# lainy/sdrangel

Measured on AMD Instinct MI355X. Metric: MS/s complex int16 IQ through decim-64 + DownChannelizer, 1/2/4/8 GPU; % HBM roofline, higher is better.
Workload: dtype int32

## Files before the change

sdrangel_amd/csrc/sdrx_chan.hip:

```cpp
#include "sdrx_common.hpp"
#include "chan_plan.hpp"
#include "tree_kernel.hpp"
#include "tree_mx_kernel.hpp"
#include <vector>
#include <cstring>
#include <new>
#include <algorithm>
#include "chan_plan.cpp"
#include "chan_lower.cpp"

using namespace sdrx;

namespace {

struct Channel {
    int32_t out_rate = 0, ofs = 0;
    int n = 0;
    uint8_t modes[32] = { 0 };
    int group = -1;
    bool passthrough = false;
    bool dead = false;
    DevBuf out;
    int64_t avail = 0;
    int64_t last_off = 0, last_n = 0;
};

struct StreamBuf {
    uint32_t* hist[2] = { nullptr, nullptr };
    int cur = 0;
    DevBuf mid;
};

struct Group {
    int index = -1;
    int64_t T = 0;
    std::vector<int> chans;
    BankPlan plan;
    LoweredBank low;
    std::vector<StreamBuf> bufs;
    void* d_static = nullptr;
    TkSubtree* d_subtrees = nullptr; TkNode* d_nodes = nullptr; TkArray* d_arrays = nullptr; TkMJob* d_mjobs = nullptr;
    TkLJob* d_ljobs = nullptr;
};

}

struct sdrx_chan_bank {
    int device = 0, cus = 256;
    int32_t in_rate = 0;
    hipStream_t own_stream = nullptr, stream = nullptr;
    std::vector<Channel> ch;
    std::vector<Group*> groups;
    DevBuf stage_in;
    DevBuf scratch;
    static constexpr int RING = 4;
    void* h_dyn[RING] = { nullptr, nullptr, nullptr, nullptr };
    void* d_dyn[RING] = { nullptr, nullptr, nullptr, nullptr };
    size_t dyn_cap[RING] = { 0, 0, 0, 0 };
    hipEvent_t dyn_ev[RING] = { nullptr, nullptr, nullptr, nullptr };
    int dyn_next = 0;
    char last_name[96] = "";
    int last_grid = 0, last_block = 0, last_lds = 0;
    EventTimer timer;
};

static void free_group(Group* g)
{
    if (!g) return;
    for (auto& s : g->bufs) { for (uint32_t* h : s.hist) if (h) (void)hipFree(h); s.mid.release(); }
    if (g->d_static) (void)hipFree(g->d_static);
    delete g;
}

static int upload_group(sdrx_chan_bank* b, Group* g)
{
    const BankPlan& p = g->plan;
    g->bufs.resize(p.streams.size());
    for (size_t si = 0; si < p.streams.size(); si++) {
        const size_t bytes = (size_t)p.streams[si].hist_len * 4;
        for (uint32_t*& h : g->bufs[si].hist) {
            SDRX_HIP(hipMalloc(reinterpret_cast<void**>(&h), bytes));
            SDRX_HIP(hipMemsetAsync(h, 0, bytes, b->stream));
        }
    }
    const size_t b0 = p.subtrees.size() * sizeof(TkSubtree), b1 = p.nodes.size() * sizeof(TkNode), b2 = p.arrays.size() * sizeof(TkArray);
    const size_t b3 = p.mjobs.size() * sizeof(TkMJob), b4 = g->low.jobs.size() * sizeof(TkLJob);
    if (b0 + b1 + b2 == 0) return SDRX_OK;
    SDRX_HIP(hipMalloc(&g->d_static, b0 + b1 + b2 + b3 + b4 + 64));
    char* d = static_cast<char*>(g->d_static);
    g->d_subtrees = reinterpret_cast<TkSubtree*>(d);
    g->d_nodes = reinterpret_cast<TkNode*>(d + b0);
    g->d_arrays = reinterpret_cast<TkArray*>(d + b0 + b1);
    g->d_mjobs = reinterpret_cast<TkMJob*>(d + b0 + b1 + b2);
    g->d_ljobs = reinterpret_cast<TkLJob*>(d + b0 + b1 + b2 + b3);
    if (b0) SDRX_HIP(hipMemcpy(g->d_subtrees, p.subtrees.data(), b0, hipMemcpyHostToDevice));
    if (b1) SDRX_HIP(hipMemcpy(g->d_nodes, p.nodes.data(), b1, hipMemcpyHostToDevice));
    if (b2) SDRX_HIP(hipMemcpy(g->d_arrays, p.arrays.data(), b2, hipMemcpyHostToDevice));
    if (b3) SDRX_HIP(hipMemcpy(g->d_mjobs, p.mjobs.data(), b3, hipMemcpyHostToDevice));
    if (b4) SDRX_HIP(hipMemcpy(g->d_ljobs, g->low.jobs.data(), b4, hipMemcpyHostToDevice));
    return SDRX_OK;
}

static int configure_channel(sdrx_chan_bank* b, int c, int32_t req_rate, int32_t req_fc)
{
    Channel& ch = b->ch[c];
    ch.n = plan_chain(b->in_rate, req_rate, req_fc, ch.modes, MAX_STAGES, &ch.out_rate, &ch.ofs);
    ch.passthrough = ch.n == 0;
    return SDRX_OK;
}

static int new_group(sdrx_chan_bank* b, const std::vector<int>& chans)
{
    if (chans.empty()) return SDRX_OK;
    std::vector<PlanChain> chains;
    for (int c : chans) chains.push_back(PlanChain{ c, b->ch[(size_t)c].n, b->ch[(size_t)c].modes });
    BankPlan plan;
    const std::string err = plan_bank(chains, plan_options_from_env(), plan);
    if (!err.empty()) { set_error(err); return SDRX_EINVAL; }
    LoweredBank low;
    (void)lower_bank(plan, low);
    Group* g = new (std::nothrow) Group;
    if (!g) return SDRX_ENOMEM;
    g->chans = chans;
    g->index = (int)b->groups.size();
    g->plan = std::move(plan);
    g->low = std::move(low);
    int rc = upload_group(b, g);
    if (rc) { free_group(g); return rc; }
    for (int c : chans) b->ch[c].group = g->index;
    b->groups.push_back(g);
    return SDRX_OK;
}

static int retire_dead_groups(sdrx_chan_bank* b)
{
    for (size_t gi = 0; gi < b->groups.size();) {
        Group* g = b->groups[gi];
        bool live = false;
        for (int c : g->chans) if (b->ch[(size_t)c].group == g->index) { live = true; break; }
        if (live) { gi++; continue; }
        SDRX_HIP(hipStreamSynchronize(b->stream));
        free_group(g);
        b->groups.erase(b->groups.begin() + (long)gi);
        for (size_t k = gi; k < b->groups.size(); k++) {
            const int old = b->groups[k]->index;
            b->groups[k]->index = (int)k;
            for (int c : b->groups[k]->chans) if (b->ch[(size_t)c].group == old) b->ch[(size_t)c].group = (int)k;
        }
    }
    return SDRX_OK;
}

static int grow_keep(sdrx_chan_bank* b, DevBuf& buf, size_t used, size_t need)
{
    if (need <= buf.cap) return SDRX_OK;
    size_t want = buf.cap ? buf.cap : (1 << 16);
    while (want < need) want *= 2;
    void* np = nullptr;
    SDRX_HIP(hipMalloc(&np, want));
    if (used) SDRX_HIP(hipMemcpyAsync(np, buf.p, used, hipMemcpyDeviceToDevice, b->stream));
    SDRX_HIP(hipStreamSynchronize(b->stream));
    if (buf.p) (void)hipFree(buf.p);
    buf.p = np; buf.cap = want;
    return SDRX_OK;
}

static int dyn_slot(sdrx_chan_bank* b, size_t bytes, int* slot)
{
    const int s = b->dyn_next; b->dyn_next = (b->dyn_next + 1) % sdrx_chan_bank::RING;
    if (b->dyn_ev[s]) SDRX_HIP(hipEventSynchronize(b->dyn_ev[s]));
    else SDRX_HIP(hipEventCreateWithFlags(&b->dyn_ev[s], hipEventDisableTiming));
    if (bytes > b->dyn_cap[s]) {
        size_t want = b->dyn_cap[s] ? b->dyn_cap[s] : 4096; while (want < bytes) want *= 2;
        if (b->h_dyn[s]) (void)hipHostFree(b->h_dyn[s]);
        if (b->d_dyn[s]) (void)hipFree(b->d_dyn[s]);
        b->h_dyn[s] = b->d_dyn[s] = nullptr; b->dyn_cap[s] = 0;
        SDRX_HIP(hipHostMalloc(&b->h_dyn[s], want, hipHostMallocDefault));
        SDRX_HIP(hipMalloc(&b->d_dyn[s], want));
        b->dyn_cap[s] = want;
    }
    *slot = s;
    return SDRX_OK;
}

static int feed_group(sdrx_chan_bank* b, Group* g, const uint32_t* d_in, int64_t n)
{
    const int64_t T0 = g->T, T1 = g->T + n;
    for (int c : g->chans) {
        Channel& ch = b->ch[c];
        if (ch.group != g->index) continue;
        const int64_t add = (T1 >> ch.n) - (T0 >> ch.n);
        int rc = grow_keep(b, ch.out, (size_t)ch.avail * 4, (size_t)(ch.avail + add) * 4 + 64); if (rc) return rc;
    }
    const BankPlan& plan = g->plan;
    for (size_t si = 1; si < plan.streams.size(); si++) {
        const int64_t add = (T1 >> plan.streams[si].depth) - (T0 >> plan.streams[si].depth);
        int rc = g->bufs[si].mid.reserve((size_t)add * 4 + 64); if (rc) return rc;
    }
    const size_t ns = plan.streams.size(), nk = plan.sinks.size();
    const size_t o_sinks = ns * sizeof(TkStream), o_hist = o_sinks + nk * sizeof(TkSink), total = o_hist + ns * sizeof(TkHistJob);
    int slot; int rc = dyn_slot(b, total, &slot); if (rc) return rc;
    char* hp = static_cast<char*>(b->h_dyn[slot]); char* dp = static_cast<char*>(b->d_dyn[slot]);
    TkStream* hs = reinterpret_cast<TkStream*>(hp);
    TkSink* hk = reinterpret_cast<TkSink*>(hp + o_sinks);
    TkHistJob* hh = reinterpret_cast<TkHistJob*>(hp + o_hist);

    std::vector<long> segs(ns, 0);
    for (size_t si = 0; si < ns; si++) {
        const PlanStream& s = plan.streams[si];
        const StreamBuf& sb = g->bufs[si];
        TkStream& t = hs[si];
        t.hist = sb.hist[sb.cur];
        t.in = si == 0 ? d_in : static_cast<const uint32_t*>(sb.mid.p);
        t.t_old = T0 >> s.depth; t.t_new = T1 >> s.depth;
        t.subtree = s.subtree;
        t.c_first = t.t_old / TK_CHUNK;
        t.c_last = t.t_new > t.t_old ? (t.t_new - 1) / TK_CHUNK : t.c_first - 1;
        t.cps = 1;
        t.hist_len = s.hist_len;
        hh[si] = TkHistJob{ sb.hist[sb.cur], t.in, sb.hist[sb.cur ^ 1], t.t_new - t.t_old, s.hist_len };
    }
    for (size_t k = 0; k < nk; k++) {
        const PlanSink& si = plan.sinks[k];
        TkSink& t = hk[k];
        t.shift = 0; t.next = si.next;
        if (si.kind == 0) {
            Channel& ch = b->ch[si.ch];
            t.lo = T0 >> si.depth; t.hi = T1 >> si.depth;
            t.ptr0 = reinterpret_cast<uint32_t*>(reinterpret_cast<uintptr_t>(ch.out.p) - (uintptr_t)(4 * (t.lo - ch.avail)));
            t.shift = si.depth;
            if (ch.group != g->index) t.hi = t.lo;
        } else {
            const int depth = plan.streams[(size_t)si.stream].depth;
            t.lo = T0 >> depth; t.hi = T1 >> depth;
            t.ptr0 = reinterpret_cast<uint32_t*>(reinterpret_cast<uintptr_t>(g->bufs[(size_t)si.stream].mid.p) - (uintptr_t)(4 * t.lo));
        }
    }
    for (const std::vector<int>& ps : plan.passes) {
        long total_chunks = 0;
        for (int si : ps) total_chunks += std::max(0L, hs[si].c_last - hs[si].c_first + 1);
        long cps = (total_chunks + (long)b->cus * 4 - 1) / ((long)b->cus * 4);
        cps = std::max(1L, std::min(cps, 256L));
        for (int si : ps) {
            hs[si].cps = (int)cps;
            segs[si] = (std::max(0L, hs[si].c_last - hs[si].c_first + 1) + cps - 1) / cps;
        }
    }
    SDRX_HIP(hipMemcpyAsync(dp, hp, total, hipMemcpyHostToDevice, b->stream));
    SDRX_HIP(hipEventRecord(b->dyn_ev[slot], b->stream));

    const TkStream* d_streams = reinterpret_cast<const TkStream*>(dp);
    const TkSink* d_sinks = reinterpret_cast<const TkSink*>(dp + o_sinks);
    const TkHistJob* d_hist = reinterpret_cast<const TkHistJob*>(dp + o_hist);
    rc = b->timer.begin(b->stream); if (rc) return rc;
    for (size_t p = 0; p < plan.passes.size(); p++) {
        const std::vector<int>& ps = plan.passes[p];
        if (ps.empty()) continue;
        long max_segs = 0;
        for (int si : ps) max_segs = std::max(max_segs, segs[si]);
        if (max_segs == 0) continue;
        const int s0 = ps.front(), cnt = (int)ps.size();
        size_t lds_bytes = 0;
        for (int si : ps) lds_bytes = std::max(lds_bytes, (size_t)plan.subtrees[(size_t)plan.streams[(size_t)si].subtree].lds_dwords * 4);
        if (g->low.pass_mx[p])
            hipLaunchKernelGGL(tree_mx_kernel, dim3((unsigned)max_segs, (unsigned)cnt), dim3(TK_THREADS), lds_bytes, b->stream,
                               g->d_subtrees, g->d_arrays, d_streams + s0, d_sinks, g->d_ljobs);
        else if (plan.mfma)
            hipLaunchKernelGGL(tree_kernel<true>, dim3((unsigned)max_segs, (unsigned)cnt), dim3(TK_THREADS), lds_bytes, b->stream,
                               g->d_subtrees, g->d_nodes, g->d_arrays, d_streams + s0, d_sinks, g->d_mjobs);
        else
            hipLaunchKernelGGL(tree_kernel<false>, dim3((unsigned)max_segs, (unsigned)cnt), dim3(TK_THREADS), lds_bytes, b->stream,
                               g->d_subtrees, g->d_nodes, g->d_arrays, d_streams + s0, d_sinks, g->d_mjobs);
        SDRX_HIP(hipGetLastError());
        if (p == 0) {
            snprintf(b->last_name, sizeof b->last_name, plan.mfma ? "tree_kernel<mfma>" : "tree_kernel<valu>");
            b->last_grid = (int)(max_segs * cnt); b->last_block = TK_THREADS; b->last_lds = (int)lds_bytes;
        }
    }
    rc = b->timer.end(b->stream); if (rc) return rc;
    long max_hist = TK_HIST;
    for (const PlanStream& s : plan.streams) max_hist = std::max(max_hist, s.hist_len);
    hipLaunchKernelGGL(tree_hist_kernel, dim3((unsigned)(max_hist / 256), (unsigned)ns), dim3(256), 0, b->stream, d_hist);
    SDRX_HIP(hipGetLastError());
    for (StreamBuf& sb : g->bufs) sb.cur ^= 1;
    for (int c : g->chans) {
        Channel& ch = b->ch[c];
        if (ch.group != g->index) continue;
        const int64_t add = (T1 >> ch.n) - (T0 >> ch.n);
        ch.last_off = ch.avail; ch.last_n = add; ch.avail += add;
    }
    g->T = T1;
    return SDRX_OK;
}

static int feed_passthrough(sdrx_chan_bank* b, const uint32_t* d_in, int64_t n)
{
    for (auto& ch : b->ch) {
        if (!ch.passthrough) continue;
        int rc = grow_keep(b, ch.out, (size_t)ch.avail * 4, (size_t)(ch.avail + n) * 4 + 64); if (rc) return rc;
        SDRX_HIP(hipMemcpyAsync(static_cast<uint32_t*>(ch.out.p) + ch.avail, d_in, (size_t)n * 4, hipMemcpyDeviceToDevice, b->stream));
        ch.last_off = ch.avail; ch.last_n = n; ch.avail += n;
    }
    return SDRX_OK;
}

extern "C" {

int sdrx_chan_plan(int32_t in_rate, int32_t req_rate, int32_t req_fc, uint8_t* modes, int32_t* out_rate, int32_t* residual_ofs)
{
    if (!modes || !out_rate || !residual_ofs) { set_error("sdrx_chan_plan: null argument"); return SDRX_EINVAL; }
    return plan_chain(in_rate, req_rate, req_fc, modes, MAX_STAGES, out_rate, residual_ofs);
}

int sdrx_chan_bank_create(sdrx_chan_bank_t** out, int device, int32_t in_rate, int32_t n_ch,
                          const int32_t* req_rate, const int32_t* req_fc)
{
    if (!out) { set_error("sdrx_chan_bank_create: null out"); return SDRX_EINVAL; }
    *out = nullptr;
    if (n_ch <= 0 || !req_rate || !req_fc || in_rate <= 0) { set_error("sdrx_chan_bank_create: bad argument"); return SDRX_EINVAL; }
    int rc = check_device(device); if (rc) return rc;
    SDRX_HIP(hipSetDevice(device));
    sdrx_chan_bank* b = new (std::nothrow) sdrx_chan_bank;
    if (!b) return SDRX_ENOMEM;
    b->device = device; b->in_rate = in_rate; b->cus = device_cu_count(device);
    hipError_t e = hipStreamCreateWithFlags(&b->own_stream, hipStreamNonBlocking);
    if (e != hipSuccess) { delete b; return hip_fail(e, "hipStreamCreate", __FILE__, __LINE__); }
    b->stream = b->own_stream;
    e = hipFuncSetAttribute(reinterpret_cast<const void*>(&tree_kernel<true>), hipFuncAttributeMaxDynamicSharedMemorySize, 160 * 1024);
    if (e == hipSuccess) e = hipFuncSetAttribute(reinterpret_cast<const void*>(&tree_kernel<false>), hipFuncAttributeMaxDynamicSharedMemorySize, 160 * 1024);
    if (e == hipSuccess) e = hipFuncSetAttribute(reinterpret_cast<const void*>(&tree_mx_kernel), hipFuncAttributeMaxDynamicSharedMemorySize, 160 * 1024);
    if (e != hipSuccess) { sdrx_chan_bank_destroy(b); return hip_fail(e, "hipFuncSetAttribute", __FILE__, __LINE__); }
    b->ch.resize((size_t)n_ch);
    std::vector<int> all;
    for (int c = 0; c < n_ch; c++) {
        configure_channel(b, c, req_rate[c], req_fc[c]);
        if (!b->ch[c].passthrough) all.push_back(c);
    }
    rc = new_group(b, all);
    if (rc) { sdrx_chan_bank_destroy(b); return rc; }
    SDRX_HIP(hipStreamSynchronize(b->stream));
    *out = b;
    return SDRX_OK;
}

int sdrx_chan_bank_destroy(sdrx_chan_bank_t* b)
{
    if (!b) return SDRX_OK;
    (void)hipSetDevice(b->device);
    if (b->stream) (void)hipStreamSynchronize(b->stream);
    for (Group* g : b->groups) free_group(g);
    for (auto& c : b->ch) c.out.release();
    b->stage_in.release(); b->scratch.release(); b->timer.release();
    for (int i = 0; i < sdrx_chan_bank::RING; i++) {
        if (b->h_dyn[i]) (void)hipHostFree(b->h_dyn[i]);
        if (b->d_dyn[i]) (void)hipFree(b->d_dyn[i]);
        if (b->dyn_ev[i]) (void)hipEventDestroy(b->dyn_ev[i]);
    }
    if (b->own_stream) (void)hipStreamDestroy(b->own_stream);
    delete b;
    return SDRX_OK;
}

int sdrx_chan_bank_info(const sdrx_chan_bank_t* b, int32_t c, int32_t* n_stages, uint8_t* modes, int32_t* out_rate, int32_t* residual_ofs)
{
    if (!b || c < 0 || c >= (int32_t)b->ch.size()) { set_error("sdrx_chan_bank_info: bad channel"); return SDRX_EINVAL; }
    const Channel& ch = b->ch[(size_t)c];
    if (n_stages) *n_stages = ch.n;
    if (modes) memcpy(modes, ch.modes, (size_t)ch.n);
    if (out_rate) *out_rate = ch.out_rate;
    if (residual_ofs) *residual_ofs = ch.ofs;
    return SDRX_OK;
}

int sdrx_chan_bank_reconfigure(sdrx_chan_bank_t* b, int32_t c, int32_t req_rate, int32_t req_fc)
{
    if (!b || c < 0 || c >= (int32_t)b->ch.size()) { set_error("sdrx_chan_bank_reconfigure: bad channel"); return SDRX_EINVAL; }
    SDRX_HIP(hipSetDevice(b->device));
    Channel& ch = b->ch[(size_t)c];
    ch.group = -1; ch.dead = false;
    configure_channel(b, c, req_rate, req_fc);
    int rc = retire_dead_groups(b); if (rc) return rc;
    if (ch.passthrough) return SDRX_OK;
    return new_group(b, std::vector<int>{ (int)c });
}

int sdrx_chan_bank_add_channel(sdrx_chan_bank_t* b, int32_t req_rate, int32_t req_fc, int32_t* channel)
{
    if (!b) { set_error("sdrx_chan_bank_add_channel: null bank"); return SDRX_EINVAL; }
    SDRX_HIP(hipSetDevice(b->device));
    b->ch.emplace_back();
    const int c = (int)b->ch.size() - 1;
    configure_channel(b, c, req_rate, req_fc);
    if (channel) *channel = c;
    if (b->ch[(size_t)c].passthrough) return SDRX_OK;
    const int rc = new_group(b, std::vector<int>{ c });
    if (rc) { b->ch.pop_back(); if (channel) *channel = -1; }
    return rc;
}

int sdrx_chan_bank_remove_channel(sdrx_chan_bank_t* b, int32_t c)
{
    if (!b || c < 0 || c >= (int32_t)b->ch.size()) { set_error("sdrx_chan_bank_remove_channel: bad channel"); return SDRX_EINVAL; }
    SDRX_HIP(hipSetDevice(b->device));
    Channel& ch = b->ch[(size_t)c];
    ch.group = -1; ch.passthrough = false; ch.dead = true; ch.n = 0; ch.out_rate = 0; ch.ofs = 0;
    ch.avail = 0; ch.last_off = 0; ch.last_n = 0;
    return retire_dead_groups(b);
}

static const int64_t CHAN_STATE_MAGIC = 0x7364727863686b31LL;

int64_t sdrx_chan_bank_state_bytes(const sdrx_chan_bank_t* b)
{
    if (!b) return SDRX_EINVAL;
    int64_t n = 16;
    for (const Group* g : b->groups) { n += 16; for (const PlanStream& s : g->plan.streams) n += 8 + (int64_t)s.hist_len * 4; }
    return n;
}

// ... 199 lines not shown
```

sdrangel_amd/csrc/tree_mx_kernel.hpp:

```cpp
#pragma once
#include "hb_common.hpp"
#include "hb_mfma.hpp"
#include "tree_layout.hpp"
#include "chan_lower.hpp"

namespace sdrx {

__device__ __forceinline__ int mx_div_pow2_trunc(int v, int n)
{
    return (v + ((v >> 31) & ((1 << n) - 1))) >> n;
}

__global__ __launch_bounds__(TK_THREADS, 4)
void tree_mx_kernel(const TkSubtree* __restrict__ subtrees, const TkArray* __restrict__ arrays, const TkStream* __restrict__ streams,
                    const TkSink* __restrict__ sinks, const TkLJob* __restrict__ ljobs)
{
    constexpr int C = TK_CHUNK, NT = TK_THREADS, LPT = C / 4 / NT;
    extern __shared__ __attribute__((aligned(16))) uint32_t lds[];

    const TkStream sp = streams[blockIdx.y];
    const long first = sp.c_first + (long)blockIdx.x * sp.cps;
    if (first > sp.c_last) return;
    long last = first + sp.cps - 1; if (last > sp.c_last) last = sp.c_last;
    const TkSubtree& st = subtrees[sp.subtree];
    const int tid = threadIdx.x;

    for (int i = tid; i < st.lds_dwords; i += NT) lds[i] = 0;
    __syncthreads();
    for (int i = tid; i < st.n_arrays * 16; i += NT) {
        const TkArray a = arrays[st.array_base + (i >> 4)];
        if (a.bias) lds[a.store + (i & 15)] = HBM_BIAS2;
    }
    typedef HbMfmaTaps<48, false> Taps;
    Taps taps;
    const int lane = tid & 63, n16 = lane & 15, g4 = lane >> 4;
    const int wv = __builtin_amdgcn_readfirstlane(tid >> 6);
    taps.init(lane);
    const uint32_t root_xm = st.root_xm;
    int n_levels = st.n_levels, store_base = st.store_base, root_off = st.root_off, root_len = st.root_len;
    asm volatile("" : "+s"(n_levels), "+s"(store_base), "+s"(root_off), "+s"(root_len));
    int rE_I = st.rootE_I, rE_Q = st.rootE_Q, rO_I = st.rootO_I, rO_Q = st.rootO_Q, rA_I = st.rootA_I, rA_Q = st.rootA_Q, root_cnt16 = st.root_arr_cnt * 16;
    asm volatile("" : "+s"(rE_I), "+s"(rE_Q), "+s"(rO_I), "+s"(rO_Q), "+s"(rA_I), "+s"(rA_Q), "+s"(root_cnt16));

    uint4 pre[LPT];
    auto fetch = [&](long chunk, const int tid) {
        const long c0 = chunk * C;
        if (c0 >= sp.t_old && c0 + C <= sp.t_new) {
            typedef uint32_t u4v __attribute__((ext_vector_type(4)));
            typedef const u4v __attribute__((address_space(1))) gq4;
            gq4* src = (gq4*)reinterpret_cast<const u4v*>(sp.in + (c0 - sp.t_old));
#pragma unroll
            for (int j = 0; j < LPT; j++) { const u4v v = src[j * NT + tid]; pre[j] = make_uint4(v[0], v[1], v[2], v[3]); }
            return;
        }
#pragma unroll
        for (int j = 0; j < LPT; j++) {
            const long p0 = chunk * C + 4 * (j * NT + tid);
            if (p0 >= sp.t_old && p0 + 4 <= sp.t_new) {
                pre[j] = *reinterpret_cast<const uint4*>(sp.in + (p0 - sp.t_old));
            } else {
                uint32_t v[4];
#pragma unroll
                for (int e = 0; e < 4; e++) {
                    const long p = p0 + e;
                    v[e] = p < sp.t_old ? sp.hist[p - (sp.t_old - sp.hist_len)] : (p < sp.t_new ? sp.in[p - sp.t_old] : 0u);
                }
                pre[j] = make_uint4(v[0], v[1], v[2], v[3]);
            }
        }
        __builtin_amdgcn_s_waitcnt(0x0F70);
    };
    fetch(first - st.warm, tid);
    __syncthreads();

    typedef int s8i __attribute__((ext_vector_type(8)));
    typedef int s16i __attribute__((ext_vector_type(16)));
    typedef unsigned short us2 __attribute__((ext_vector_type(2)));
    const v4i bias = { Taps::BIAS, Taps::BIAS, Taps::BIAS, Taps::BIAS };
    const char* ldsb = reinterpret_cast<const char*>(lds);
    char* ldsw = reinterpret_cast<char*>(lds);
    const int wl = 32 * n16 + 16 * g4, cl = 32 * n16 + 8 * g4, pl = 16 * n16 + 4 * g4;
    constexpr uint32_t PLAIN = 0x00010001u, ALT = 0x0001ffffu;
    auto padd = [](uint32_t a, uint32_t b) { return __builtin_bit_cast(uint32_t, (us2)(__builtin_bit_cast(us2, a) + __builtin_bit_cast(us2, b))); };
    auto psub = [](uint32_t a, uint32_t b) { return __builtin_bit_cast(uint32_t, (us2)(__builtin_bit_cast(us2, a) - __builtin_bit_cast(us2, b))); };
    auto pmul = [](uint32_t a, uint32_t m) { return __builtin_bit_cast(uint32_t, (us2)(__builtin_bit_cast(us2, a) * __builtin_bit_cast(us2, m))); };

    for (long chunk = first - st.warm; chunk <= last; ++chunk) {
        int tid = threadIdx.x;
        asm volatile("" : "+v"(tid));
#pragma unroll
        for (int j = 0; j < LPT; j++) {
            const int q = HIST / 2 + j * NT + tid;
            const uint4 v = pre[j];
            const uint32_t oI = __builtin_amdgcn_perm(v.w, v.y, 0x05040100u);
            const uint32_t oQ = __builtin_amdgcn_perm(v.w, v.y, 0x07060302u);
            lds[rE_I + q] = __builtin_amdgcn_perm(v.z, v.x, 0x05040100u);
            lds[rE_Q + q] = __builtin_amdgcn_perm(v.z, v.x, 0x07060302u);
            if (rO_I >= 0) { lds[rO_I + q] = oI ^ root_xm; lds[rO_Q + q] = oQ ^ root_xm; }
            if (rA_I >= 0) { lds[rA_I + q] = pmul(oI, ALT) ^ root_xm; lds[rA_Q + q] = pmul(oQ, ALT) ^ root_xm; }
        }
        for (int i = tid; i < root_cnt16; i += NT)
            lds[root_off + (i >> 4) * root_len + (i & 15)] = lds[store_base + i];
        if (chunk < last) fetch(chunk + 1, tid);
        __syncthreads();

        const bool live = chunk >= first;
        int lv0 = 0;
        asm volatile("" : "+s"(lv0), "+s"(n_levels));
        auto level = [&](auto Lc) {
            constexpr int L = decltype(Lc)::value;
            constexpr int PI = mx_pitch(L), PO = mx_pitch(L + 1);
            const s16i rec = *(const s16i __attribute__((address_space(4)))*)reinterpret_cast<const int*>(&st.lv[L + lv0]);
            const int nout = rec[3], arr_base = rec[4], arr_cnt = rec[5], in_len = rec[7], mjob_base = rec[9], n_mjobs = rec[10];
            const uint32_t xm = (uint32_t)rec[11];
            const int prev_off = rec[12], prev_arr_cnt = rec[13], arr_off = rec[14], arr_len = rec[15];
            {
                const int n_restore = arr_cnt * 16, n_all = n_restore + prev_arr_cnt * 16;
                const int slot0 = store_base + 16 * arr_base;
                for (int i = tid; i < n_all; i += NT) {
                    const int k = i - n_restore;
                    const int src = k < 0 ? slot0 + i : prev_off + (k >> 4) * in_len + in_len - 16 + (k & 15);
                    const int dst = k < 0 ? arr_off + (i >> 4) * arr_len + (i & 15) : slot0 - prev_arr_cnt * 16 + k;
                    lds[dst] = lds[src];
                }
            }
            struct JobIn { v4i bI0, bI1, bQ0, bQ1; uint2 cI01, cQ01; uint32_t cI2, cQ2; };
            auto load = [&](const s8i d, JobIn& r, auto Cc) {
                const char* pb = ldsb + d[0] + wl;
                r.bI0 = *reinterpret_cast<const v4i*>(__builtin_assume_aligned(pb, 16));
                r.bI1 = *reinterpret_cast<const v4i*>(__builtin_assume_aligned(pb + 64, 16));
                r.bQ0 = *reinterpret_cast<const v4i*>(__builtin_assume_aligned(pb + PI, 16));
                r.bQ1 = *reinterpret_cast<const v4i*>(__builtin_assume_aligned(pb + PI + 64, 16));
                const char* pc = ldsb + d[1] + cl;
                const char *pI, *pQ;
                if constexpr (decltype(Cc)::value == MX_FAST) { pI = pc + PI; pQ = pc; }
                else { const bool lu = d[7] & MX_LU_BIT; pI = lu ? pc + PI : pc; pQ = lu ? pc : pc + PI; }
                r.cI01 = *reinterpret_cast<const uint2*>(__builtin_assume_aligned(pI, 8));
                r.cI2 = *reinterpret_cast<const uint32_t*>(pI + 8);
                r.cQ01 = *reinterpret_cast<const uint2*>(__builtin_assume_aligned(pQ, 8));
                r.cQ2 = *reinterpret_cast<const uint32_t*>(pQ + 8);
            };
            auto st32 = [&](char* p, int off, uint32_t v) { *reinterpret_cast<uint32_t*>(p + off) = v; };
            auto child = [&](auto Sk, const uint32_t eI, const uint32_t oI, const uint32_t eQ, const uint32_t oQ, const int base, const int f,
                             const int sink, const long abs0) {
                constexpr bool SINK = decltype(Sk)::value;
                if (f) {
                    char* p = ldsw + base + pl;
                    const uint32_t m = (f & 2) ? PLAIN : ALT;
                    st32(p, 0, eI); st32(p, PO, eQ);
                    st32(p, 2 * PO, pmul(oI, m) ^ xm); st32(p, 3 * PO, pmul(oQ, m) ^ xm);
                    if (f == 7) { st32(p, 4 * PO, pmul(oI, ALT) ^ xm); st32(p, 5 * PO, pmul(oQ, ALT) ^ xm); }
                }
                if constexpr (SINK) {
                    if (live) {
                        typedef const s8i __attribute__((address_space(4))) cs8;
                        for (int si = sink; si >= 0; ) {
                            const s8i sr = *(cs8*)reinterpret_cast<const int*>(sinks + si);
                            const long ptr0 = ((long)sr[1] << 32) | (uint32_t)sr[0];
                            const long lo = ((long)sr[3] << 32) | (uint32_t)sr[2], hi = ((long)sr[5] << 32) | (uint32_t)sr[4];
                            const int shift = sr[6];
                            uint32_t w[4];
                            if (shift) {
                                w[0] = pack_iq(mx_div_pow2_trunc((int)(int16_t)eI, shift), mx_div_pow2_trunc((int)(int16_t)eQ, shift));
                                w[1] = pack_iq(mx_div_pow2_trunc((int)(int16_t)oI, shift), mx_div_pow2_trunc((int)(int16_t)oQ, shift));
                                w[2] = pack_iq(mx_div_pow2_trunc((int)eI >> 16, shift), mx_div_pow2_trunc((int)eQ >> 16, shift));
                                w[3] = pack_iq(mx_div_pow2_trunc((int)oI >> 16, shift), mx_div_pow2_trunc((int)oQ >> 16, shift));
                            } else {
                                w[0] = __builtin_amdgcn_perm(eQ, eI, 0x05040100u); w[1] = __builtin_amdgcn_perm(oQ, oI, 0x05040100u);
                                w[2] = __builtin_amdgcn_perm(eQ, eI, 0x07060302u); w[3] = __builtin_amdgcn_perm(oQ, oI, 0x07060302u);
                            }
                            typedef uint32_t __attribute__((address_space(1))) gu32;
                            gu32* dst = (gu32*)(reinterpret_cast<uint32_t*>(ptr0) + abs0);
                            const long rel = abs0 - lo, span = hi - lo;
                            if (rel >= 0 && rel + 4 <= span) {
                                typedef uint32_t u4a __attribute__((ext_vector_type(4), aligned(4)));
                                *(u4a __attribute__((address_space(1)))*)dst = u4a{ w[0], w[1], w[2], w[3] };
                            } else if (rel > -4 && rel < span) {
#pragma unroll
                                for (int i = 0; i < 4; i++) if (rel + i >= 0 && rel + i < span) dst[i] = w[i];
                            }
                            si = sr[7];
                        }
                    }
                }
            };
            auto finish = [&](auto Cc, const JobIn& r, const v4i SI, const v4i SQ, const s8i d) {
                constexpr int CLS = decltype(Cc)::value;
                auto shpack = [](int a, int b) {
                    uint32_t v = (uint32_t)(a >> (HB_SHIFT - 1));
                    asm("v_ashrrev_i32_sdwa %0, %1, %2 dst_sel:WORD_1 dst_unused:UNUSED_PRESERVE src0_sel:DWORD src1_sel:DWORD" : "+v"(v) : "s"(HB_SHIFT - 1), "v"(b));
                    return v;
                };
                const uint32_t sI02 = shpack(SI[0], SI[2]), sI13 = shpack(SI[1], SI[3]);
                const uint32_t sQ02 = shpack(SQ[0], SQ[2]), sQ13 = shpack(SQ[1], SQ[3]);
                const uint32_t cI02 = __builtin_amdgcn_perm(r.cI01.y, r.cI01.x, 0x07060302u), cI13 = __builtin_amdgcn_perm(r.cI2, r.cI01.y, 0x05040100u);
                const uint32_t cQ02 = __builtin_amdgcn_perm(r.cQ01.y, r.cQ01.x, 0x07060302u), cQ13 = __builtin_amdgcn_perm(r.cQ2, r.cQ01.y, 0x05040100u);
                const int meta = d[7], f0 = (meta >> 4) & 15, f1 = (meta >> 8) & 15;
                if constexpr (CLS == MX_FAST) {
                    const uint32_t ma = (f0 & 2) ? PLAIN : ALT, mb = (f1 & 2) ? PLAIN : ALT;
                    auto st4 = [&](const int base, uint32_t eI, uint32_t eQ, uint32_t oI, uint32_t oQ, uint32_t m) {
                        char* p = ldsw + base + pl;
                        st32(p, 0, eI); st32(p, PO, eQ); st32(p, 2 * PO, pmul(oI, m) ^ xm); st32(p, 3 * PO, pmul(oQ, m) ^ xm);
                    };
                    st4(d[2], padd(sI02, cI02), psub(sQ02, cQ02), psub(sI13, cI13), padd(sQ13, cQ13), ma);
                    st4(d[3], psub(sI02, cI02), padd(sQ02, cQ02), padd(sI13, cI13), psub(sQ13, cQ13), mb);
                } else {
                    const std::integral_constant<bool, CLS == MX_SINK> Sk;
                    const long abs0 = CLS == MX_SINK ? chunk * nout + d[6] + 16 * n16 + 4 * g4 : 0;
                    const uint32_t sg = (meta & MX_LU_BIT) ? 0xffffffffu : PLAIN;
                    if (f0 | (d[4] >= 0)) {
                        const uint32_t nI13 = pmul(cI13, sg), nQ02 = pmul(cQ02, sg);
                        child(Sk, padd(sI02, cI02), padd(sI13, nI13), padd(sQ02, nQ02), padd(sQ13, cQ13), d[2], f0, d[4], abs0);
                    }
                    if (f1 | (d[5] >= 0)) child(Sk, psub(sI02, cI02), padd(sI13, cI13), padd(sQ02, cQ02), psub(sQ13, cQ13), d[3], f1, d[5], abs0);
                }
            };
            auto pair = [&](auto Cc, const s8i d0, const s8i d1) {
                JobIn r0, r1;
                __builtin_amdgcn_s_setprio(2);
                load(d0, r0, Cc); load(d1, r1, Cc);
                __builtin_amdgcn_sched_barrier(0);
                const v4i SI0 = taps.tile(r0.bI0, r0.bI1, bias), SQ0 = taps.tile(r0.bQ0, r0.bQ1, bias);
                const v4i SI1 = taps.tile(r1.bI0, r1.bI1, bias), SQ1 = taps.tile(r1.bQ0, r1.bQ1, bias);
                __builtin_amdgcn_s_setprio(0);
                finish(Cc, r0, SI0, SQ0, d0);
                finish(Cc, r1, SI1, SQ1, d1);
            };
            auto single = [&](auto Cc, const s8i d0) {
                JobIn r0;
                load(d0, r0, Cc);
                const v4i SI0 = taps.tile(r0.bI0, r0.bI1, bias), SQ0 = taps.tile(r0.bQ0, r0.bQ1, bias);
                finish(Cc, r0, SI0, SQ0, d0);
            };
            typedef std::integral_constant<int, MX_FAST> KF;
            typedef std::integral_constant<int, MX_ARMS> KA;
            typedef std::integral_constant<int, MX_SINK> KS;
            const int per = (n_mjobs + NT / 64 - 1) / (NT / 64);
            const int t0 = wv * per, t1 = t0 + per < n_mjobs ? t0 + per : n_mjobs;
            typedef const s8i __attribute__((address_space(4))) cs8j;
            for (int tt = t0; tt < t1; ) {
                const s8i d0 = *(cs8j*)reinterpret_cast<const int*>(ljobs + mjob_base + tt);
                const int c0 = d0[7] & 15;
                if (tt + 1 < t1) {
                    const s8i d1 = *(cs8j*)reinterpret_cast<const int*>(ljobs + mjob_base + tt + 1);
                    if ((d1[7] & 15) == c0) {
                        if (c0 == MX_FAST) pair(KF{}, d0, d1);
                        else if (c0 == MX_ARMS) pair(KA{}, d0, d1);
                        else pair(KS{}, d0, d1);
                        tt += 2;
                        continue;
                    }
                }
                if (c0 == MX_FAST) single(KF{}, d0);
                else if (c0 == MX_ARMS) single(KA{}, d0);
                else single(KS{}, d0);
                tt += 1;
            }
            __syncthreads();
        };
        level(std::integral_constant<int, 0>{});
        if (n_levels > 1) level(std::integral_constant<int, 1>{});
        if (n_levels > 2) level(std::integral_constant<int, 2>{});
        if (n_levels > 3) level(std::integral_constant<int, 3>{});
    }
}

}
```

Before: 249,200.

## Compile per-wave job programs into LDS for the MX tree kernel

```diff
diff --git a/sdrangel_amd/csrc/chan_prog.cpp b/sdrangel_amd/csrc/chan_prog.cpp
--- /dev/null
+++ b/sdrangel_amd/csrc/chan_prog.cpp
@@ -0,0 +1,120 @@
+#include "chan_prog.hpp"
+#include "chan_plan.hpp"
+#include <algorithm>
+
+namespace sdrx {
+
+namespace {
+
+bool fits16(long v) { return v >= 0 && v < 65536; }
+
+std::string subtree_program(const TkSubtree& st, const LoweredBank& low, int lds, int sink_lds, std::vector<uint32_t>& w)
+{
+    w.assign(PROG_DIR_DW, 0);
+    for (int wave = 0; wave < PROG_WAVES; wave++) {
+        w[(size_t)wave] = (uint32_t)(lds * 4 + (int)w.size() * 4);
+        for (int l = 0; l < st.n_levels; l++) {
+            const TkLevel& lv = st.lv[l];
+            if (lv.nout != TK_CHUNK >> (l + 1)) return "program: level with another output count";
+            if (lv.xm != 0 && lv.xm != HBM_BIAS2) return "program: unexpected odd-arm bias";
+            const long slot0 = st.store_base + 16L * lv.arr_base - 16L * lv.prev_arr_cnt, n_save = 16L * lv.prev_arr_cnt;
+            const long n_all = n_save + 16L * lv.arr_cnt, tail = (long)lv.prev_off + lv.in_len - 16;
+            if (!fits16(slot0) || !fits16(n_all) || !fits16(tail) || lv.arr_off < 0) return "program: history walk outside 16 bits";
+            const int per = (lv.n_mjobs + PROG_WAVES - 1) / PROG_WAVES;
+            const int t0 = std::min(wave * per, lv.n_mjobs), t1 = std::min(t0 + per, lv.n_mjobs);
+            int cnt[MX_CLASSES] = { 0 };
+            for (int t = t0; t < t1; t++) cnt[mx_class(low.jobs[(size_t)(lv.mjob_base + t)].meta)]++;
+            if (cnt[0] > 255 || cnt[1] > 255 || cnt[2] > 255) return "program: too many jobs for one wave";
+            w.push_back((uint32_t)(slot0 | n_save << 16));
+            w.push_back((uint32_t)(tail | n_all << 16));
+            w.push_back((uint32_t)lv.arr_off);
+            w.push_back((uint32_t)(cnt[0] | cnt[1] << 8 | cnt[2] << 16 | (lv.xm ? 1 : 0) << 24));
+            for (int t = t0; t < t1; t++) {
+                const TkLJob& j = low.jobs[(size_t)(lv.mjob_base + t)];
+                if (t > t0 && mx_class(j.meta) < mx_class(low.jobs[(size_t)(lv.mjob_base + t - 1)].meta)) return "program: jobs not sorted by class";
+                if (!fits16(j.b) || !fits16(j.c) || !fits16(j.o[0]) || !fits16(j.o[1])) return "program: job address outside 16 bits";
+                w.push_back((uint32_t)j.b | (uint32_t)j.c << 16);
+                w.push_back((uint32_t)j.o[0] | (uint32_t)j.o[1] << 16);
+                if (mx_class(j.meta) == MX_FAST) {
+                    w.push_back((mx_flags(j.meta, 0) & 2) ? PROG_PLAIN : PROG_ALT);
+                    w.push_back((mx_flags(j.meta, 1) & 2) ? PROG_PLAIN : PROG_ALT);
+                } else {
+                    uint32_t sk = 0;
+                    for (int k = 0; k < 2; k++) {
+                        if (j.sink[k] < 0) continue;
+                        const long a = sink_lds < 0 ? 1 : 4L * sink_lds + 4L * TK_SINK_DW * (j.sink[k] - st.sink_base);
+                        if (j.sink[k] < st.sink_base || j.sink[k] >= st.sink_base + st.n_sinks || !fits16(a) || a == 0) return "program: sink outside the subtree's run";
+                        sk |= (uint32_t)a << (16 * k);
+                    }
+                    if ((j.out0 & 255) || j.out0 < 0 || j.out0 >= TK_CHUNK) return "program: first output not a whole job";
+                    w.push_back(sk);
+                    w.push_back((uint32_t)((j.meta & (0xff0 | MX_LU_BIT)) | (j.out0 >> 8) << 20));
+                }
+            }
+        }
+    }
+    w.insert(w.end(), PROG_PAD_DW, 0u);
+    return {};
+}
+
+}
+
+std::string build_programs(const BankPlan& plan, const LoweredBank& low, ProgBank& out)
+{
+    out = ProgBank{};
+    out.sub.assign(plan.subtrees.size(), TkProg{ 0, 0, 0, 0 });
+    out.pass_ok.assign(plan.passes.size(), 0);
+    out.pass_lds.assign(plan.passes.size(), 0);
+    std::string first_err;
+    for (size_t p = 0; p < plan.passes.size(); p++) {
+        int base = 0;
+        for (int si : plan.passes[p]) {
+            const int s = plan.streams[(size_t)si].subtree;
+            if (s >= 0) base = std::max(base, plan.subtrees[(size_t)s].lds_dwords * 4);
+        }
+        out.pass_lds[p] = base;
+        if (p >= low.pass_mx.size() || !low.pass_mx[p] || base <= 0) continue;
+        std::string err;
+        int need = base;
+        const size_t words0 = out.words.size();
+        std::vector<std::pair<int, TkProg>> made;
+        for (int si : plan.passes[p]) {
+            const int s = plan.streams[(size_t)si].subtree;
+            const TkSubtree& st = plan.subtrees[(size_t)s];
+            if (std::any_of(made.begin(), made.end(), [s](const std::pair<int, TkProg>& m) { return m.first == s; })) continue;
+            for (int k = st.sink_base; k < st.sink_base + st.n_sinks && err.empty(); k++) {
+                const int nx = k < (int)plan.sinks.size() ? plan.sinks[(size_t)k].next : st.sink_base - 1;
+                if (nx != -1 && (nx < st.sink_base || nx >= st.sink_base + st.n_sinks)) err = "program: sink list leaves the subtree's run";
+            }
+            if (!err.empty()) break;
+            std::vector<uint32_t> w;
+            int lds = (st.node_tab + 3) & ~3;
+            for (int tries = 0; tries < 2; tries++) {
+                err = subtree_program(st, low, lds, -1, w);
+                if (!err.empty()) break;
+                const int sink_lds = (lds + (int)w.size() + 3) & ~3, end = sink_lds + st.n_sinks * TK_SINK_DW;
+                if (tries == 0 && end > st.lds_dwords) { lds = (st.lds_dwords + 3) & ~3; continue; }
+                err = subtree_program(st, low, lds, sink_lds, w);
+                if (err.empty()) {
+                    need = std::max(need, end * 4);
+                    made.emplace_back(s, TkProg{ (int)out.words.size(), (int)w.size(), lds, sink_lds });
+                    out.words.insert(out.words.end(), w.begin(), w.end());
+                }
+                break;
+            }
+            if (!err.empty()) break;
+        }
+        if (err.empty() && (need > PROG_LDS_MAX || PROG_LDS_MAX / need != PROG_LDS_MAX / base)) err = "program: no room in LDS without losing a workgroup per CU";
+        if (!err.empty()) {
+            out.words.resize(words0);
+            if (first_err.empty()) first_err = err;
+            continue;
+        }
+        for (const auto& m : made) out.sub[(size_t)m.first] = m.second;
+        out.pass_ok[p] = 1;
+        out.pass_lds[p] = need;
+    }
+    return first_err;
+}
+
+}
diff --git a/sdrangel_amd/csrc/chan_prog.hpp b/sdrangel_amd/csrc/chan_prog.hpp
--- /dev/null
+++ b/sdrangel_amd/csrc/chan_prog.hpp
@@ -0,0 +1,30 @@
+#pragma once
+#include "chan_lower.hpp"
+#include <string>
+#include <vector>
+
+namespace sdrx {
+
+constexpr int PROG_WAVES = TK_THREADS / 64;
+constexpr int PROG_ITEM = 16;
+constexpr int PROG_DIR_DW = 4, PROG_PAD_DW = 12;
+constexpr uint32_t PROG_PLAIN = 0x00010001u, PROG_ALT = 0x0001ffffu;
+constexpr int PROG_LDS_MAX = 160 * 1024;
+
+struct TkProg {
+    int src;
+    int dwords;
+    int lds;
+    int sinks;
+};
+
+struct ProgBank {
+    std::vector<uint32_t> words;
+    std::vector<TkProg> sub;
+    std::vector<uint8_t> pass_ok;
+    std::vector<int> pass_lds;
+};
+
+std::string build_programs(const BankPlan& plan, const LoweredBank& low, ProgBank& out);
+
+}
diff --git a/sdrangel_amd/csrc/sdrx_chan.hip b/sdrangel_amd/csrc/sdrx_chan.hip
--- a/sdrangel_amd/csrc/sdrx_chan.hip
+++ b/sdrangel_amd/csrc/sdrx_chan.hip
@@ -8,6 +8,7 @@
 #include <algorithm>
 #include "chan_plan.cpp"
 #include "chan_lower.cpp"
+#include "chan_prog.cpp"
 
 using namespace sdrx;
 
@@ -36,11 +37,11 @@
     int64_t T = 0;
     std::vector<int> chans;
     BankPlan plan;
-    LoweredBank low;
+    ProgBank prog;
     std::vector<StreamBuf> bufs;
     void* d_static = nullptr;
     TkSubtree* d_subtrees = nullptr; TkNode* d_nodes = nullptr; TkArray* d_arrays = nullptr; TkMJob* d_mjobs = nullptr;
-    TkLJob* d_ljobs = nullptr;
+    TkProg* d_progs = nullptr; uint32_t* d_prog_words = nullptr;
 };
 
 }
@@ -84,20 +85,22 @@
         }
     }
     const size_t b0 = p.subtrees.size() * sizeof(TkSubtree), b1 = p.nodes.size() * sizeof(TkNode), b2 = p.arrays.size() * sizeof(TkArray);
-    const size_t b3 = p.mjobs.size() * sizeof(TkMJob), b4 = g->low.jobs.size() * sizeof(TkLJob);
+    const size_t b3 = p.mjobs.size() * sizeof(TkMJob), b4 = g->prog.sub.size() * sizeof(TkProg), b5 = g->prog.words.size() * 4;
     if (b0 + b1 + b2 == 0) return SDRX_OK;
-    SDRX_HIP(hipMalloc(&g->d_static, b0 + b1 + b2 + b3 + b4 + 64));
+    SDRX_HIP(hipMalloc(&g->d_static, b0 + b1 + b2 + b3 + b4 + b5 + 64));
     char* d = static_cast<char*>(g->d_static);
     g->d_subtrees = reinterpret_cast<TkSubtree*>(d);
     g->d_nodes = reinterpret_cast<TkNode*>(d + b0);
     g->d_arrays = reinterpret_cast<TkArray*>(d + b0 + b1);
     g->d_mjobs = reinterpret_cast<TkMJob*>(d + b0 + b1 + b2);
-    g->d_ljobs = reinterpret_cast<TkLJob*>(d + b0 + b1 + b2 + b3);
+    g->d_progs = reinterpret_cast<TkProg*>(d + b0 + b1 + b2 + b3);
+    g->d_prog_words = reinterpret_cast<uint32_t*>(d + b0 + b1 + b2 + b3 + b4);
     if (b0) SDRX_HIP(hipMemcpy(g->d_subtrees, p.subtrees.data(), b0, hipMemcpyHostToDevice));
     if (b1) SDRX_HIP(hipMemcpy(g->d_nodes, p.nodes.data(), b1, hipMemcpyHostToDevice));
     if (b2) SDRX_HIP(hipMemcpy(g->d_arrays, p.arrays.data(), b2, hipMemcpyHostToDevice));
     if (b3) SDRX_HIP(hipMemcpy(g->d_mjobs, p.mjobs.data(), b3, hipMemcpyHostToDevice));
-    if (b4) SDRX_HIP(hipMemcpy(g->d_ljobs, g->low.jobs.data(), b4, hipMemcpyHostToDevice));
+    if (b4) SDRX_HIP(hipMemcpy(g->d_progs, g->prog.sub.data(), b4, hipMemcpyHostToDevice));
+    if (b5) SDRX_HIP(hipMemcpy(g->d_prog_words, g->prog.words.data(), b5, hipMemcpyHostToDevice));
     return SDRX_OK;
 }
 
@@ -119,12 +122,14 @@
     if (!err.empty()) { set_error(err); return SDRX_EINVAL; }
     LoweredBank low;
     (void)lower_bank(plan, low);
+    ProgBank prog;
+    (void)build_programs(plan, low, prog);
     Group* g = new (std::nothrow) Group;
     if (!g) return SDRX_ENOMEM;
     g->chans = chans;
     g->index = (int)b->groups.size();
     g->plan = std::move(plan);
-    g->low = std::move(low);
+    g->prog = std::move(prog);
     int rc = upload_group(b, g);
     if (rc) { free_group(g); return rc; }
     for (int c : chans) b->ch[c].group = g->index;
@@ -260,11 +265,10 @@
         for (int si : ps) max_segs = std::max(max_segs, segs[si]);
         if (max_segs == 0) continue;
         const int s0 = ps.front(), cnt = (int)ps.size();
-        size_t lds_bytes = 0;
-        for (int si : ps) lds_bytes = std::max(lds_bytes, (size_t)plan.subtrees[(size_t)plan.streams[(size_t)si].subtree].lds_dwords * 4);
-        if (g->low.pass_mx[p])
+        const size_t lds_bytes = (size_t)g->prog.pass_lds[p];
+        if (g->prog.pass_ok[p])
             hipLaunchKernelGGL(tree_mx_kernel, dim3((unsigned)max_segs, (unsigned)cnt), dim3(TK_THREADS), lds_bytes, b->stream,
-                               g->d_subtrees, g->d_arrays, d_streams + s0, d_sinks, g->d_ljobs);
+                               g->d_subtrees, g->d_arrays, d_streams + s0, d_sinks, g->d_progs, g->d_prog_words);
         else if (plan.mfma)
             hipLaunchKernelGGL(tree_kernel<true>, dim3((unsigned)max_segs, (unsigned)cnt), dim3(TK_THREADS), lds_bytes, b->stream,
                                g->d_subtrees, g->d_nodes, g->d_arrays, d_streams + s0, d_sinks, g->d_mjobs);
diff --git a/sdrangel_amd/csrc/tree_mx_kernel.hpp b/sdrangel_amd/csrc/tree_mx_kernel.hpp
--- a/sdrangel_amd/csrc/tree_mx_kernel.hpp
+++ b/sdrangel_amd/csrc/tree_mx_kernel.hpp
@@ -3,6 +3,7 @@
 #include "hb_mfma.hpp"
 #include "tree_layout.hpp"
 #include "chan_lower.hpp"
+#include "chan_prog.hpp"
 
 namespace sdrx {
 
@@ -13,7 +14,7 @@
 
 __global__ __launch_bounds__(TK_THREADS, 4)
 void tree_mx_kernel(const TkSubtree* __restrict__ subtrees, const TkArray* __restrict__ arrays, const TkStream* __restrict__ streams,
-                    const TkSink* __restrict__ sinks, const TkLJob* __restrict__ ljobs)
+                    const TkSink* __restrict__ sinks, const TkProg* __restrict__ progs, const uint32_t* __restrict__ prog_words)
 {
     constexpr int C = TK_CHUNK, NT = TK_THREADS, LPT = C / 4 / NT;
     extern __shared__ __attribute__((aligned(16))) uint32_t lds[];
@@ -27,6 +28,16 @@
 
     for (int i = tid; i < st.lds_dwords; i += NT) lds[i] = 0;
     __syncthreads();
+    const TkProg pg = progs[sp.subtree];
+    for (int i = tid; i < pg.dwords; i += NT) lds[pg.lds + i] = prog_words[pg.src + i];
+    {
+        const uint32_t* sk = reinterpret_cast<const uint32_t*>(sinks + st.sink_base);
+        for (int i = tid; i < st.n_sinks * TK_SINK_DW; i += NT) {
+            uint32_t v = sk[i];
+            if ((i & 7) == 7) v = (int)v < 0 ? 0u : (uint32_t)(4 * pg.sinks + 4 * TK_SINK_DW * ((int)v - st.sink_base));
+            lds[pg.sinks + i] = v;
+        }
+    }
     for (int i = tid; i < st.n_arrays * 16; i += NT) {
         const TkArray a = arrays[st.array_base + (i >> 4)];
         if (a.bias) lds[a.store + (i & 15)] = HBM_BIAS2;
@@ -38,6 +49,7 @@
     taps.init(lane);
     const uint32_t root_xm = st.root_xm;
     int n_levels = st.n_levels, store_base = st.store_base, root_off = st.root_off, root_len = st.root_len;
+    const int prog_dir = pg.lds;
     asm volatile("" : "+s"(n_levels), "+s"(store_base), "+s"(root_off), "+s"(root_len));
     int rE_I = st.rootE_I, rE_Q = st.rootE_Q, rO_I = st.rootO_I, rO_Q = st.rootO_Q, rA_I = st.rootA_I, rA_Q = st.rootA_Q, root_cnt16 = st.root_arr_cnt * 16;
     asm volatile("" : "+s"(rE_I), "+s"(rE_Q), "+s"(rO_I), "+s"(rO_Q), "+s"(rA_I), "+s"(rA_Q), "+s"(root_cnt16));
@@ -72,12 +84,15 @@
     };
     fetch(first - st.warm, tid);
     __syncthreads();
-
-    typedef int s8i __attribute__((ext_vector_type(8)));
-    typedef int s16i __attribute__((ext_vector_type(16)));
+    auto rfl = [](uint32_t v) { return (uint32_t)__builtin_amdgcn_readfirstlane((int)v); };
+    uint32_t pstart = rfl(lds[prog_dir + wv]);
+    asm volatile("" : "+s"(pstart));
+
     typedef unsigned short us2 __attribute__((ext_vector_type(2)));
     const v4i bias = { Taps::BIAS, Taps::BIAS, Taps::BIAS, Taps::BIAS };
     const char* ldsb = reinterpret_cast<const char*>(lds);
+    auto ldsq = [&](uint32_t a) { return *reinterpret_cast<const uint4*>(__builtin_assume_aligned(ldsb + a, 16)); };
+    auto lds32 = [&](uint32_t a) { return *reinterpret_cast<const uint32_t*>(ldsb + a); };
     char* ldsw = reinterpret_cast<char*>(lds);
     const int wl = 32 * n16 + 16 * g4, cl = 32 * n16 + 8 * g4, pl = 16 * n16 + 4 * g4;
     constexpr uint32_t PLAIN = 0x00010001u, ALT = 0x0001ffffu;
@@ -102,50 +117,58 @@
         for (int i = tid; i < root_cnt16; i += NT)
             lds[root_off + (i >> 4) * root_len + (i & 15)] = lds[store_base + i];
         if (chunk < last) fetch(chunk + 1, tid);
+        uint32_t pp = pstart;
+        uint4 hdr = ldsq(pp);
+        uint32_t nb0 = lds32(pp + PROG_ITEM), nb1 = lds32(pp + 2 * PROG_ITEM);
         __syncthreads();
 
         const bool live = chunk >= first;
-        int lv0 = 0;
-        asm volatile("" : "+s"(lv0), "+s"(n_levels));
         auto level = [&](auto Lc) {
             constexpr int L = decltype(Lc)::value;
-            constexpr int PI = mx_pitch(L), PO = mx_pitch(L + 1);
-            const s16i rec = *(const s16i __attribute__((address_space(4)))*)reinterpret_cast<const int*>(&st.lv[L + lv0]);
-            const int nout = rec[3], arr_base = rec[4], arr_cnt = rec[5], in_len = rec[7], mjob_base = rec[9], n_mjobs = rec[10];
-            const uint32_t xm = (uint32_t)rec[11];
-            const int prev_off = rec[12], prev_arr_cnt = rec[13], arr_off = rec[14], arr_len = rec[15];
-            {
-                const int n_restore = arr_cnt * 16, n_all = n_restore + prev_arr_cnt * 16;
-                const int slot0 = store_base + 16 * arr_base;
-                for (int i = tid; i < n_all; i += NT) {
-                    const int k = i - n_restore;
-                    const int src = k < 0 ? slot0 + i : prev_off + (k >> 4) * in_len + in_len - 16 + (k & 15);
-                    const int dst = k < 0 ? arr_off + (i >> 4) * arr_len + (i & 15) : slot0 - prev_arr_cnt * 16 + k;
-                    lds[dst] = lds[src];
-                }
-            }
+            constexpr int PI = mx_pitch(L), PO = mx_pitch(L + 1), NOUT = C >> (L + 1);
+            const uint32_t h0 = rfl(hdr.x), h1 = rfl(hdr.y), ctl = rfl(hdr.w);
+            const int arr_off = (int)rfl(hdr.z);
+            const uint32_t xm = (ctl >> 24) ? HBM_BIAS2 : 0u;
+            pp += PROG_ITEM;
+            const int n_all = (int)(h1 >> 16);
+            int wk = 0;
+            auto walk_addr = [&](const int m, const bool src) {
+                const int n_save = (int)(h0 >> 16), slot = (int)(h0 & 0xffffu) + m;
+                const bool save = m < n_save;
+                const int k = save ? m : m - n_save;
+                const int win = (save ? (int)(h1 & 0xffffu) : arr_off) + (int)__umul24((uint32_t)k >> 4, save ? PI / 4 : PO / 4) + (k & 15);
+                return save == src ? win : slot;
+            };
+            auto walk_load = [&](uint32_t& v) { const int m = wk + tid; if (m < n_all) v = lds[walk_addr(m, true)]; };
+            auto walk_store = [&](const uint32_t v) {
+                int t = tid;
+                asm volatile("" : "+v"(t));
+                const int m = wk + t;
+                if (m < n_all) lds[walk_addr(m, false)] = v;
+                wk += NT;
+            };
             struct JobIn { v4i bI0, bI1, bQ0, bQ1; uint2 cI01, cQ01; uint32_t cI2, cQ2; };
-            auto load = [&](const s8i d, JobIn& r, auto Cc) {
-                const char* pb = ldsb + d[0] + wl;
+            auto load = [&](const uint32_t bc, const bool lu, JobIn& r, auto Cc) {
+                const char* pb = ldsb + ((bc & 0xffffu) + wl);
                 r.bI0 = *reinterpret_cast<const v4i*>(__builtin_assume_aligned(pb, 16));
                 r.bI1 = *reinterpret_cast<const v4i*>(__builtin_assume_aligned(pb + 64, 16));
                 r.bQ0 = *reinterpret_cast<const v4i*>(__builtin_assume_aligned(pb + PI, 16));
                 r.bQ1 = *reinterpret_cast<const v4i*>(__builtin_assume_aligned(pb + PI + 64, 16));
-                const char* pc = ldsb + d[1] + cl;
+                const char* pc = ldsb + ((bc >> 16) + cl);
                 const char *pI, *pQ;
                 if constexpr (decltype(Cc)::value == MX_FAST) { pI = pc + PI; pQ = pc; }
-                else { const bool lu = d[7] & MX_LU_BIT; pI = lu ? pc + PI : pc; pQ = lu ? pc : pc + PI; }
+                else { pI = lu ? pc + PI : pc; pQ = lu ? pc : pc + PI; }
                 r.cI01 = *reinterpret_cast<const uint2*>(__builtin_assume_aligned(pI, 8));
                 r.cI2 = *reinterpret_cast<const uint32_t*>(pI + 8);
                 r.cQ01 = *reinterpret_cast<const uint2*>(__builtin_assume_aligned(pQ, 8));
                 r.cQ2 = *reinterpret_cast<const uint32_t*>(pQ + 8);
             };
             auto st32 = [&](char* p, int off, uint32_t v) { *reinterpret_cast<uint32_t*>(p + off) = v; };
-            auto child = [&](auto Sk, const uint32_t eI, const uint32_t oI, const uint32_t eQ, const uint32_t oQ, const int base, const int f,
-                             const int sink, const long abs0) {
+            auto child = [&](auto Sk, const uint32_t eI, const uint32_t oI, const uint32_t eQ, const uint32_t oQ, const uint32_t base, const int f,
+                             const uint32_t sink, const long abs0) {
                 constexpr bool SINK = decltype(Sk)::value;
                 if (f) {
-                    char* p = ldsw + base + pl;
+                    char* p = ldsw + (base + pl);
                     const uint32_t m = (f & 2) ? PLAIN : ALT;
                     st32(p, 0, eI); st32(p, PO, eQ);
                     st32(p, 2 * PO, pmul(oI, m) ^ xm); st32(p, 3 * PO, pmul(oQ, m) ^ xm);
@@ -153,12 +176,11 @@
                 }
                 if constexpr (SINK) {
                     if (live) {
-                        typedef const s8i __attribute__((address_space(4))) cs8;
-                        for (int si = sink; si >= 0; ) {
-                            const s8i sr = *(cs8*)reinterpret_cast<const int*>(sinks + si);
-                            const long ptr0 = ((long)sr[1] << 32) | (uint32_t)sr[0];
-                            const long lo = ((long)sr[3] << 32) | (uint32_t)sr[2], hi = ((long)sr[5] << 32) | (uint32_t)sr[4];
-                            const int shift = sr[6];
+                        for (uint32_t si = sink; si; ) {
+                            const uint4 sa = ldsq(si), sb = ldsq(si + 16);
+                            const long ptr0 = ((long)sa.y << 32) | sa.x;
+                            const long lo = ((long)sa.w << 32) | sa.z, hi = ((long)sb.y << 32) | sb.x;
+                            const int shift = (int)rfl(sb.z);
                             uint32_t w[4];
                             if (shift) {
                                 w[0] = pack_iq(mx_div_pow2_trunc((int)(int16_t)eI, shift), mx_div_pow2_trunc((int)(int16_t)eQ, shift));
@@ -179,12 +201,12 @@
 #pragma unroll
                                 for (int i = 0; i < 4; i++) if (rel + i >= 0 && rel + i < span) dst[i] = w[i];
                             }
-                            si = sr[7];
+                            si = rfl(sb.w);
                         }
                     }
                 }
             };
-            auto finish = [&](auto Cc, const JobIn& r, const v4i SI, const v4i SQ, const s8i d) {
+            auto finish = [&](auto Cc, const JobIn& r, const v4i SI, const v4i SQ, const uint4 d, const int meta) {
                 constexpr int CLS = decltype(Cc)::value;
                 auto shpack = [](int a, int b) {
                     uint32_t v = (uint32_t)(a >> (HB_SHIFT - 1));
@@ -195,67 +217,70 @@
                 const uint32_t sQ02 = shpack(SQ[0], SQ[2]), sQ13 = shpack(SQ[1], SQ[3]);
                 const uint32_t cI02 = __builtin_amdgcn_perm(r.cI01.y, r.cI01.x, 0x07060302u), cI13 = __builtin_amdgcn_perm(r.cI2, r.cI01.y, 0x05040100u);
                 const uint32_t cQ02 = __builtin_amdgcn_perm(r.cQ01.y, r.cQ01.x, 0x07060302u), cQ13 = __builtin_amdgcn_perm(r.cQ2, r.cQ01.y, 0x05040100u);
-                const int meta = d[7], f0 = (meta >> 4) & 15, f1 = (meta >> 8) & 15;
                 if constexpr (CLS == MX_FAST) {
-                    const uint32_t ma = (f0 & 2) ? PLAIN : ALT, mb = (f1 & 2) ? PLAIN : ALT;
-                    auto st4 = [&](const int base, uint32_t eI, uint32_t eQ, uint32_t oI, uint32_t oQ, uint32_t m) {
-                        char* p = ldsw + base + pl;
+                    auto st4 = [&](const uint32_t base, uint32_t eI, uint32_t eQ, uint32_t oI, uint32_t oQ, uint32_t m) {
+                        char* p = ldsw + (base + pl);
                         st32(p, 0, eI); st32(p, PO, eQ); st32(p, 2 * PO, pmul(oI, m) ^ xm); st32(p, 3 * PO, pmul(oQ, m) ^ xm);
                     };
-                    st4(d[2], padd(sI02, cI02), psub(sQ02, cQ02), psub(sI13, cI13), padd(sQ13, cQ13), ma);
-                    st4(d[3], psub(sI02, cI02), padd(sQ02, cQ02), padd(sI13, cI13), psub(sQ13, cQ13), mb);
+                    st4(d.y & 0xffffu, padd(sI02, cI02), psub(sQ02, cQ02), psub(sI13, cI13), padd(sQ13, cQ13), d.z);
+                    st4(d.y >> 16, psub(sI02, cI02), padd(sQ02, cQ02), padd(sI13, cI13), psub(sQ13, cQ13), d.w);
                 } else {
                     const std::integral_constant<bool, CLS == MX_SINK> Sk;
-                    const long abs0 = CLS == MX_SINK ? chunk * nout + d[6] + 16 * n16 + 4 * g4 : 0;
+                    const int f0 = (meta >> 4) & 15, f1 = (meta >> 8) & 15;
+                    const uint32_t sk = CLS == MX_SINK ? rfl(d.z) : 0u, sk0 = sk & 0xffffu, sk1 = sk >> 16;
+                    const long abs0 = CLS == MX_SINK ? chunk * NOUT + (((meta >> 20) & 15) << 8) + 16 * n16 + 4 * g4 : 0;
                     const uint32_t sg = (meta & MX_LU_BIT) ? 0xffffffffu : PLAIN;
-                    if (f0 | (d[4] >= 0)) {
+                    if (f0 | (int)sk0) {
                         const uint32_t nI13 = pmul(cI13, sg), nQ02 = pmul(cQ02, sg);
-                        child(Sk, padd(sI02, cI02), padd(sI13, nI13), padd(sQ02, nQ02), padd(sQ13, cQ13), d[2], f0, d[4], abs0);
+                        child(Sk, padd(sI02, cI02), padd(sI13, nI13), padd(sQ02, nQ02), padd(sQ13, cQ13), d.y & 0xffffu, f0, sk0, abs0);
                     }
-                    if (f1 | (d[5] >= 0)) child(Sk, psub(sI02, cI02), padd(sI13, cI13), padd(sQ02, cQ02), psub(sQ13, cQ13), d[3], f1, d[5], abs0);
-                }
-            };
-            auto pair = [&](auto Cc, const s8i d0, const s8i d1) {
+                    if (f1 | (int)sk1) child(Sk, psub(sI02, cI02), padd(sI13, cI13), padd(sQ02, cQ02), psub(sQ13, cQ13), d.y >> 16, f1, sk1, abs0);
+                }
+            };
+            auto pair = [&](auto Cc) {
+                constexpr bool F = decltype(Cc)::value == MX_FAST;
                 JobIn r0, r1;
+                const uint4 d0 = ldsq(pp), d1 = ldsq(pp + PROG_ITEM);
+                const int m0 = F ? 0 : (int)rfl(d0.w), m1 = F ? 0 : (int)rfl(d1.w);
                 __builtin_amdgcn_s_setprio(2);
-                load(d0, r0, Cc); load(d1, r1, Cc);
+                load(nb0, m0 & MX_LU_BIT, r0, Cc); load(nb1, m1 & MX_LU_BIT, r1, Cc);
+                uint32_t wv_ = 0;
+                const bool walk = wk < n_all;
+                if (walk) walk_load(wv_);
                 __builtin_amdgcn_sched_barrier(0);
                 const v4i SI0 = taps.tile(r0.bI0, r0.bI1, bias), SQ0 = taps.tile(r0.bQ0, r0.bQ1, bias);
                 const v4i SI1 = taps.tile(r1.bI0, r1.bI1, bias), SQ1 = taps.tile(r1.bQ0, r1.bQ1, bias);
                 __builtin_amdgcn_s_setprio(0);
-                finish(Cc, r0, SI0, SQ0, d0);
-                finish(Cc, r1, SI1, SQ1, d1);
-            };
-            auto single = [&](auto Cc, const s8i d0) {
+                pp += 2 * PROG_ITEM;
+                nb0 = lds32(pp); nb1 = lds32(pp + PROG_ITEM);
+                if (walk) walk_store(wv_);
+                finish(Cc, r0, SI0, SQ0, d0, m0);
+                finish(Cc, r1, SI1, SQ1, d1, m1);
+            };
+            auto single = [&](auto Cc) {
+                constexpr bool F = decltype(Cc)::value == MX_FAST;
                 JobIn r0;
-                load(d0, r0, Cc);
+                const uint4 d0 = ldsq(pp);
+                const int m0 = F ? 0 : (int)rfl(d0.w);
+                load(nb0, m0 & MX_LU_BIT, r0, Cc);
+                uint32_t wv_ = 0;
+                const bool walk = wk < n_all;
+                if (walk) walk_load(wv_);
                 const v4i SI0 = taps.tile(r0.bI0, r0.bI1, bias), SQ0 = taps.tile(r0.bQ0, r0.bQ1, bias);
-                finish(Cc, r0, SI0, SQ0, d0);
-            };
-            typedef std::integral_constant<int, MX_FAST> KF;
-            typedef std::integral_constant<int, MX_ARMS> KA;
-            typedef std::integral_constant<int, MX_SINK> KS;
-            const int per = (n_mjobs + NT / 64 - 1) / (NT / 64);
-            const int t0 = wv * per, t1 = t0 + per < n_mjobs ? t0 + per : n_mjobs;
-            typedef const s8i __attribute__((address_space(4))) cs8j;
-            for (int tt = t0; tt < t1; ) {
-                const s8i d0 = *(cs8j*)reinterpret_cast<const int*>(ljobs + mjob_base + tt);
-                const int c0 = d0[7] & 15;
-                if (tt + 1 < t1) {
-                    const s8i d1 = *(cs8j*)reinterpret_cast<const int*>(ljobs + mjob_base + tt + 1);
-                    if ((d1[7] & 15) == c0) {
-                        if (c0 == MX_FAST) pair(KF{}, d0, d1);
-                        else if (c0 == MX_ARMS) pair(KA{}, d0, d1);
-                        else pair(KS{}, d0, d1);
-                        tt += 2;
-                        continue;
-                    }
-                }
-                if (c0 == MX_FAST) single(KF{}, d0);
-                else if (c0 == MX_ARMS) single(KA{}, d0);
-                else single(KS{}, d0);
-                tt += 1;
-            }
+                pp += PROG_ITEM;
+                nb0 = nb1; nb1 = lds32(pp + PROG_ITEM);
+                if (walk) walk_store(wv_);
+                finish(Cc, r0, SI0, SQ0, d0, m0);
+            };
+            auto run = [&](auto Cc, int n) {
+                for (; n >= 2; n -= 2) pair(Cc);
+                if (n) single(Cc);
+            };
+            run(std::integral_constant<int, MX_FAST>{}, (int)(ctl & 255u));
+            run(std::integral_constant<int, MX_ARMS>{}, (int)((ctl >> 8) & 255u));
+            run(std::integral_constant<int, MX_SINK>{}, (int)((ctl >> 16) & 255u));
+            while (wk < n_all) { uint32_t v = 0; walk_load(v); walk_store(v); }
+            hdr = ldsq(pp); nb0 = lds32(pp + PROG_ITEM); nb1 = lds32(pp + 2 * PROG_ITEM);
             __syncthreads();
         };
         level(std::integral_constant<int, 0>{});
```

After: 234,100. 0.939x the previous value.
